# vLAR-group/unMORE

Hardware: NVIDIA B200
Metric: object_reasoning_images_per_sec (higher is better)
Workload: dtype f32

## Files before the change

include/unmore_b200.h:

```cpp
#ifndef UNMORE_B200_H_
#define UNMORE_B200_H_

#include <stddef.h>
#include <stdint.h>

#ifdef __cplusplus
extern "C" {
#endif

#define UNMORE_E_INVALID (-1)
#define UNMORE_E_CAPACITY (-2)

typedef void* unmore_stream_t;

const char* unmore_last_error(void);
int unmore_version(void);
size_t unmore_workspace_bytes(int n_img);

int unmore_existence_scores(const float* fields, int n_img, int C, int H, int W, int ch_exist,
                            const void* boxes, int boxes_f64, const int* counts, int cap,
                            float* scores_out, void* ws, unmore_stream_t stream);

int unmore_crop_resize(const float* fields, int n_img, int C, int H, int W,
                       const int* channels_host, int n_channels, const void* boxes, int boxes_f64,
// ... 16 lines not shown
                                     float max_sdf_thres, float max_shrink_threshold, float delta_ratio,
                                     float* boxes_out, float* labels_out, float* deltas_ws, float* max_ws,
                                     unmore_stream_t stream);
int unmore_score_and_rasterise_from_tiles(const float* tiles, const float* existence_scores, int antialias,
                                          int n_img, int H, int W, const void* boxes, int boxes_f64,
                                          const int* counts, int cap, float* scores_out, float* tight_out,
                                          int* areas_out, uint32_t* masks_out, unmore_stream_t stream);

int unmore_center_reasoning(const float* fields, int n_img, int C, int H, int W, int ch_sdf,
                            int ch_center_row, int ch_center_col, const void* boxes, int boxes_f64,
                            const int* counts, int cap, double center_score_max_thres,
                            double* max_values_out, int* argmax_out, double* splits_out,
                            unsigned char* cc_counts_out, double* cc_boxes_out, int* cc_overflow,
                            void* ws, unmore_stream_t stream);
int unmore_cc_cap(void);

int unmore_boundary_refine(const float* fields, int n_img, int C, int H, int W, int ch_sdf,
                           const void* boxes, int boxes_f64, const int* counts, int cap, int n_round,
                           int apply_small_filter, int early_exit, float proposal_area_thres,
                           float max_sdf_thres, float max_shrink_threshold, float delta_ratio,
                           float* boxes_out, float* labels_out, int* rounds_out, void* ws,
                           unmore_stream_t stream);

int unmore_existence_scores_aa(const float* fields, int n_img, int C, int H, int W, int ch_exist,
                               const void* boxes, int boxes_f64, const int* counts, int cap,
                               float* scores_out, void* ws, unmore_stream_t stream);
int unmore_boundary_refine_aa(const float* fields, int n_img, int C, int H, int W, int ch_sdf,
                              const void* boxes, int boxes_f64, const int* counts, int cap, int n_round,
                              int apply_small_filter, int early_exit, float proposal_area_thres,
                              float max_sdf_thres, float max_shrink_threshold, float delta_ratio,
// ... 74 lines not shown
```

unmore_b200/_lib.py:

```python
from __future__ import annotations

import ctypes as C
import os

_HERE = os.path.dirname(os.path.abspath(__file__))
LIB_PATH = os.environ.get("UNMORE_B200_LIB", os.path.join(_HERE, "libunmore_b200.so"))

_p = C.c_void_p
_i = C.c_int
_f = C.c_float
_d = C.c_double

SIGNATURES = {
    "unmore_existence_scores": [_p, _i, _i, _i, _i, _i, _p, _i, _p, _i, _p, _p, _p],
    "unmore_existence_scores_aa": [_p, _i, _i, _i, _i, _i, _p, _i, _p, _i, _p, _p, _p],
    "unmore_crop_resize": [_p, _i, _i, _i, _i, _p, _i, _p, _i, _p, _i, _p, _p],
    "unmore_crop_resize_aa": [_p, _i, _i, _i, _i, _p, _i, _p, _i, _p, _i, _p, _p, C.c_size_t, _p],
    "unmore_mask_resize_aa": [_p, _i, _i, _i, _i, _i, _p, _p, C.c_size_t, _p],
    "unmore_tile_means": [_p, C.c_longlong, _i, _p, _p],
    "unmore_center_reasoning_from_tiles": [_p, _i, _i, _i, _p, _i, _p, _i, _d, _p, _p, _p, _p, _p, _p, _p, _p],
    "unmore_boundary_round_from_tiles": [_p, _i, _p, _i, _i, _i, _f, _f, _f, _p, _p, _p, _p, _p],
    "unmore_score_and_rasterise_from_tiles": [_p, _p, _i, _i, _i, _i, _p, _i, _p, _i, _p, _p, _p, _p, _p],
    "unmore_center_reasoning": [_p, _i, _i, _i, _i, _i, _i, _i, _p, _i, _p, _i, _d, _p, _p, _p, _p, _p, _p, _p, _p],
    "unmore_boundary_refine": [_p, _i, _i, _i, _i, _i, _p, _i, _p, _i, _i, _i, _i, _f, _f, _f, _f, _p, _p, _p, _p, _p],
    "unmore_boundary_refine_aa": [_p, _i, _i, _i, _i, _i, _p, _i, _p, _i, _i, _i, _i, _f, _f, _f, _f, _p, _p, _p, _p, _p],
    "unmore_update_bbox_from_tiles": [_p, _i, _p, _p, _p],
    "unmore_compact_boxes": [_p, _i, _p, _i, _i, _i, _p, _f, _p, _i, _i, _p, _i, _p, _p, _p, _i, _p],
    "unmore_box_nms": [_p, _p, _p, _i, _i, _f, _p, _p, _p, _p, _p],
    "unmore_batch_erode": [_p, _i, _i, _i, _i, _i, _p, _p],
    "unmore_connected_components": [_p, _i, _i, _i, _p, _p, _p],
    "unmore_anti_center_map": [_p, _i, _i, _i, _i, _p, _p],
    "unmore_box_nms_matrix": [_p, _p, _i, _f, _p, _p, _p, _p, _p],
    "unmore_score_and_rasterise": [_p, _i, _i, _i, _i, _i, _i, _i, _i, _p, _i, _p, _i, _p, _p, _p, _p, _p],
    "unmore_mask_resize": [_p, _i, _i, _i, _i, _i, _p, _p],
    "unmore_final_scores": [_p, _p, _p, _p, _p, _i, _i, _d, _d, _d, _p, _p, _p, _p],
    "unmore_pack_detections": [_p, _p, _p, _p, _i, _i, _p, _i, _p],
    "unmore_sat_build": [_p, _i, _i, _i, _p, _p],
    "unmore_sat_build_fields": [_p, _i, _i, _i, _i, _p, _i, _p, _p],
# ... 43 lines not shown
```

unmore_b200/csrc/capi.cu:

```cuda
#include <cstdio>
#include <cstdarg>
#include <cmath>
#include <cstring>

#include "../../include/unmore_b200.h"
#include "unmore_internal.h"

using namespace unmore;

namespace {

thread_local char g_err[512] = "";

int fail(int code, const char* fmt, ...) {
  va_list ap;
  va_start(ap, fmt);
  vsnprintf(g_err, sizeof(g_err), fmt, ap);
  va_end(ap);
  return code;
}

int cuda_fail(int code, const char* what) {
  if (code == 0) return 0;
  snprintf(g_err, sizeof(g_err), "%s: %s", what, cudaGetErrorString((cudaError_t)code));
// ... 96 lines not shown
  if (int e = make_worklist(p.work, counts, n_img, cap, ws, s)) return e;
  if (W <= kWindowMaxSide && H <= kWindowMaxSide) {
    p.windows = window_tables(ws, n_img);
    const int e = (int)cudaMemsetAsync(p.windows, 0, sizeof(WindowSlot) * kWindowSlots * (size_t)n_img, s);
    if (e) return cuda_fail(e, "memset window tables");
  }
  if (aa) return cuda_fail(launch_refine_aa(p, num_sms(), s), "refine_aa_kernel");
  return cuda_fail(launch_refine(p, num_sms(), s), "refine_kernel");
}

}

extern "C" {

const char* unmore_last_error(void) { return g_err; }
int unmore_version(void) { return 101; }
size_t unmore_workspace_bytes(int n_img) {
  return worklist_bytes(n_img) + (n_img > 0 ? alignof(WindowSlot) - 1 + sizeof(WindowSlot) * kWindowSlots * (size_t)n_img : 0);
}

int unmore_existence_scores(const float* fields, int n_img, int C, int H, int W, int ch_exist, const void* boxes,
                            int boxes_f64, const int* counts, int cap, float* scores_out, void* ws,
                            unmore_stream_t stream) {
  return existence_scores("unmore_existence_scores", false, fields, n_img, C, H, W, ch_exist, boxes, boxes_f64, counts, cap,
                          scores_out, ws, (cudaStream_t)stream);
}

int unmore_existence_scores_aa(const float* fields, int n_img, int C, int H, int W, int ch_exist, const void* boxes,
                               int boxes_f64, const int* counts, int cap, float* scores_out, void* ws,
                               unmore_stream_t stream) {
  return existence_scores("unmore_existence_scores_aa", true, fields, n_img, C, H, W, ch_exist, boxes, boxes_f64, counts, cap,
// ... 49 lines not shown
      ch_center_row >= C || ch_center_col < 0 || ch_center_col >= C)
    return fail(UNMORE_E_INVALID, "unmore_center_reasoning: bad argument");
  if (cap == 0) return 0;
  cudaStream_t s = (cudaStream_t)stream;
  CenterParams p{};
  p.fields = fields; p.C = C; p.H = H; p.W = W;
  p.ch_sdf = ch_sdf; p.ch_crow = ch_center_row; p.ch_ccol = ch_center_col;
  p.boxes = boxes; p.boxes_f64 = boxes_f64; p.thr = center_score_max_thres;
  p.max_values = max_values_out; p.argmax = argmax_out; p.splits = splits_out;
  if ((cc_counts_out != nullptr) != (cc_boxes_out != nullptr) || (cc_counts_out != nullptr) != (cc_overflow != nullptr))
    return fail(UNMORE_E_INVALID, "unmore_center_reasoning: the three analyze_cc outputs go together");
  p.cc_counts = cc_counts_out; p.cc_boxes = cc_boxes_out; p.cc_overflow = cc_overflow;
  center_filters(p);
  if (int e = make_worklist(p.work, counts, n_img, cap, ws, s)) return e;
  return cuda_fail(launch_center(p, num_sms(), s), "center_kernel");
}

int unmore_boundary_refine(const float* fields, int n_img, int C, int H, int W, int ch_sdf, const void* boxes,
                           int boxes_f64, const int* counts, int cap, int n_round, int apply_small_filter,
                           int early_exit, float proposal_area_thres, float max_sdf_thres, float max_shrink_threshold,
                           float delta_ratio, float* boxes_out, float* labels_out, int* rounds_out, void* ws,
                           unmore_stream_t stream) {
  return boundary_refine("unmore_boundary_refine", false, fields, n_img, C, H, W, ch_sdf, boxes, boxes_f64, counts, cap, n_round,
                         apply_small_filter, early_exit, proposal_area_thres, max_sdf_thres, max_shrink_threshold,
                         delta_ratio, boxes_out, labels_out, rounds_out, ws, (cudaStream_t)stream);
}

int unmore_boundary_refine_aa(const float* fields, int n_img, int C, int H, int W, int ch_sdf, const void* boxes,
                              int boxes_f64, const int* counts, int cap, int n_round, int apply_small_filter,
                              int early_exit, float proposal_area_thres, float max_sdf_thres, float max_shrink_threshold,
// ... 249 lines not shown
```

unmore_b200/csrc/center.cu:

```cuda
#include "resample.cuh"
#include "unmore_internal.h"

namespace unmore {

constexpr int kCenterThreads = 256;
constexpr int kCenterWarps = kCenterThreads / 32;
constexpr int kWinLo = 10, kWinHi = 118, kWin = kWinHi - kWinLo;
constexpr int kWinStride = 110;
constexpr int kErode = 12;
constexpr int kCandCap = 1024;

struct CenterSmem {
  float2 c[kWin * kWinStride];
  uint32_t mask[kCrop][4];
  uint32_t hrun[kCrop][4];
  uint32_t ero[kCrop][4];
  double red_val[kCenterWarps];
  int red_idx[kCenterWarps];
  float red_f[kCenterWarps];
  float red_m[kCenterWarps];
  int bcast_i[2];
  int cc_scan[kCenterWarps];
  int cand_n;
  uint16_t cand[kCandCap];
// ... 158 lines not shown
};

struct CenterTileRows {
  const float* tile;
  __device__ __forceinline__ void row(int lane, int i, float s[4], f32x2 ab[4]) const {
    const float* r = tile + i * kCrop + lane;
#pragma unroll
    for (int c = 0; c < 4; ++c) {
      s[c] = __ldg(r + 32 * c);
      ab[c] = pk2(__ldg(r + kCrop * kCrop + 32 * c), __ldg(r + 2 * kCrop * kCrop + 32 * c));
    }
  }
};

constexpr int kSpecPlaneElems = 480 * 640;
template <bool ANALYZE_CC, int PLANE_ELEMS, bool ROW_SKIP>
__global__ void __launch_bounds__(kCenterThreads, 2) center_kernel(const CenterParams p) {
  extern __shared__ __align__(16) unsigned char smem_raw[];
  CenterSmem& sm = *reinterpret_cast<CenterSmem*>(smem_raw);
  struct WorkItem { int id, img, k, pad; double box[4]; };
  __shared__ __align__(16) WorkItem s_item[2];
  const int tid = threadIdx.x, lane = tid & 31, warp = tid >> 5;
  const int total = worklist_total(p.work);
  auto fetch_box = [&](int slot, int fimg, int fk) {
    const size_t frow = (size_t)fimg * p.work.cap + fk;
    const unsigned dst = smem_addr(&s_item[slot].box[0]);
    if (p.boxes_f64) {
      const char* src = reinterpret_cast<const char*>(p.boxes) + frow * 32;
      asm volatile("cp.async.ca.shared.global [%0], [%1], 16;" ::"r"(dst), "l"(src) : "memory");
      asm volatile("cp.async.ca.shared.global [%0], [%1], 16;" ::"r"(dst + 16), "l"(src + 16) : "memory");
    } else {
// ... 53 lines not shown
      const float scale_y = __fdiv_rn((float)win.h(), (float)kCrop);
      const int in_h = win.h();
      float cabs = 0.f;
      const bool col_in[4] = {lane >= kWinLo, true, true, lane + 96 < kWinHi};
      constexpr bool kLattice = ROW_SKIP && !ANALYZE_CC && PLANE_ELEMS >= 0;
      constexpr int kLatFirst = 8, kLatStride = 16, kLatRows = kCrop / kLatStride;
      constexpr int kRowsPerWarp = (kCrop + kCenterWarps - 1) / kCenterWarps;
      int i_begin, i_end, i_step;
      if constexpr (kLattice) { i_begin = kLatFirst + kLatStride * warp; i_end = kCrop; i_step = kLatStride * kCenterWarps; }
      else { i_begin = warp * kRowsPerWarp; i_end = min(kCrop, i_begin + kRowsPerWarp); i_step = 1; }
      int rmin = kErode, rmax = kCrop - kErode - 1;
      bool no_survivors = false;
      const unsigned stage_base = smem_addr(&sm.c[0]) + (unsigned)(((0 - kWinLo) * kWinStride + (lane - kWinLo)) * 8);
      const unsigned mask_base = smem_addr(&sm.mask[0][0]);
      const bool lane0 = lane == 0;
#pragma unroll 1
      for (int phase = 0; phase < (kLattice ? 2 : 1); ++phase) {
        const AxisTap my_tap = axis_tap(scale_y, min(i_begin + lane * i_step, kCrop - 1), in_h);
        int j = 0;
        for (int i = i_begin; i < i_end; i += i_step, ++j) {
          if (kLattice && phase == 1 && (i & (kLatStride - 1)) == kLatFirst) continue;
          const bool row_in = i >= kWinLo && i < kWinHi;
          const unsigned stage_addr = stage_base + (unsigned)(i * (kWinStride * 8));
          const unsigned mask_addr = mask_base + 16u * (unsigned)i;
          AxisTap v;
          v.i0 = __shfl_sync(kFullMask, my_tap.i0, j);
          v.l1 = __shfl_sync(kFullMask, my_tap.l1, j);
          v.i1 = min(v.i0 + 1, in_h - 1);
          v.l0 = __fsub_rn(1.f, v.l1);
          float s[4];
          f32x2 ab[4];
          if constexpr (PLANE_ELEMS < 0) trows.row(lane, i, s, ab);
          else rows.row(taps, v, s, ab);
          uint32_t word[4];
#pragma unroll
          for (int c = 0; c < 4; ++c) {
            float a2, b2;
            upk2(mul2(ab[c], ab[c]), a2, b2);
            const float sq = __fadd_rn(a2, b2);
            const bool on = (s[c] > UNMORE_SIGMOID_HALF_THRESHOLD) || (sq > UNMORE_NORM_HALF_SQ_THRESHOLD);
            word[c] = __ballot_sync(kFullMask, on);
            cabs = fmaxf(cabs, sq);
          }
          st_shared_b32_if<0>(lane0, mask_addr, word[0]);
          st_shared_b32_if<4>(lane0, mask_addr, word[1]);
          st_shared_b32_if<8>(lane0, mask_addr, word[2]);
          st_shared_b32_if<12>(lane0, mask_addr, word[3]);
          st_shared_b64_if<0>(row_in && col_in[0], stage_addr, ab[0]);
          st_shared_b64_if<256>(row_in, stage_addr, ab[1]);
          st_shared_b64_if<512>(row_in, stage_addr, ab[2]);
          st_shared_b64_if<768>(row_in && col_in[3], stage_addr, ab[3]);
        }
        if (kLattice && phase == 0) {
          __syncthreads();
          bool alive_row = false;
          if (lane < kLatRows) {
            u128 m = load_row(sm.mask[kLatFirst + kLatStride * lane]);
            m &= m >> 1; m &= m >> 2; m &= m >> 4; m &= m >> 8; m &= m >> 9;
            alive_row = m != 0;
          }
          const unsigned alive = __ballot_sync(kFullMask, alive_row);
          unsigned long long klo = 0, khi = 0;
#pragma unroll
          for (int k = 0; k < kLatRows; ++k) {
            const int l = kLatFirst + kLatStride * k, a = l - kErode < 0 ? 0 : l - kErode, b = l + kErode > kCrop - 1 ? kCrop - 1 : l + kErode;
            unsigned long long lo = 0, hi = 0;
// ... 20 lines not shown
        m &= m >> 1; m &= m >> 2; m &= m >> 4; m &= m >> 8;
        m &= m >> 9;
        store_row(sm.hrun[tid], m << kErode);
      }
      __syncthreads();
      if (tid < kCrop) {
        u128 e = 0;
        if (tid >= rmin && tid <= rmax) {
          e = ~(u128)0;
#pragma unroll 5
          for (int d = -kErode; d <= kErode; ++d) e &= load_row(sm.hrun[tid + d]);
        }
        store_row(sm.ero[tid], e);
      }
      __syncthreads();
      constexpr int kInner = kCrop - 2 * kErode;
      constexpr int kStrips = kInner / 8;
      constexpr int kMaxOwn = (kInner * kStrips + kCenterThreads - 1) / kCenterThreads;
      float own_max[kMaxOwn];
      auto strip_bits = [&](int r, int k) -> uint32_t {
        const int c = kErode + 8 * k;
        const uint32_t lo = sm.ero[r][c >> 5], hi = sm.ero[r][min((c >> 5) + 1, 3)];
        return (__funnelshift_r(lo, hi, c & 31)) & 0xffu;
      };
      auto strip_scores = [&](int r, int k, float acc[8]) {
        f32x2 acc2[8];
#pragma unroll
        for (int x = 0; x < 8; ++x) acc2[x] = pk2(0.f, 0.f);
        const int c = kErode + 8 * k;
#pragma unroll
        for (int di = 0; di < 5; ++di) {
          const int o = (r + di - 2 - kWinLo) * kWinStride + (c - 2 - kWinLo);
          f32x2 v[12];
#pragma unroll
          for (int q2 = 0; q2 < 6; ++q2) {
            const ulonglong2 t = *reinterpret_cast<const ulonglong2*>(&sm.c[o + 2 * q2]);
            v[2 * q2] = t.x; v[2 * q2 + 1] = t.y;
          }
#pragma unroll
          for (int dj = 0; dj < 5; ++dj) {
            if (di == 2 && dj == 2) continue;
            const f32x2 f = p.filt_pair[di * 5 + dj];
#pragma unroll
            for (int x = 0; x < 8; ++x) acc2[x] = fma2(f, v[x + dj], acc2[x]);
          }
        }
#pragma unroll
        for (int x = 0; x < 8; ++x) {
          float lo, hi;
          upk2(acc2[x], lo, hi);
          acc[x] = lo + hi;
        }
      };
      float m32 = -INFINITY;
#pragma unroll
      for (int m = 0; m < kMaxOwn; ++m) {
        own_max[m] = -INFINITY;
        const int q = tid + m * kCenterThreads;
        if (q < kInner * kStrips) {
          const int r = kErode + q % kInner, k = q / kInner;
          const uint32_t bits = strip_bits(r, k);
          if (bits) {
            float acc[8];
            strip_scores(r, k, acc);
#pragma unroll
            for (int x = 0; x < 8; ++x)
              if ((bits >> x) & 1u) own_max[m] = fmaxf(own_max[m], acc[x]);
            m32 = fmaxf(m32, own_max[m]);
// ... 19 lines not shown
        if (!any_cand || !(own_max[m] >= cand_thr)) continue;
        const int q = tid + m * kCenterThreads;
        const int r = kErode + q % kInner, k = q / kInner;
        const uint32_t bits = strip_bits(r, k);
        float acc[8];
        strip_scores(r, k, acc);
#pragma unroll
        for (int x = 0; x < 8; ++x) {
          if (((bits >> x) & 1u) && acc[x] >= cand_thr) {
            const int slot = atomicAdd(&sm.cand_n, 1);
            if (slot < kCandCap) sm.cand[slot] = (uint16_t)(r * kCrop + kErode + 8 * k + x);
          }
        }
      }
      __syncthreads();
      auto exact = [&](int r, int c) -> double {
        double e = 0.0;
#pragma unroll
        for (int di = 0; di < 5; ++di) {
#pragma unroll
          for (int dj = 0; dj < 5; ++dj) {
            if (di == 2 && dj == 2) continue;
            const float2 cc = sm.c[(r + di - 2 - kWinLo) * kWinStride + (c + dj - 2 - kWinLo)];
            e = fma(p.filt[di * 5 + dj], (double)cc.x, e);
            e = fma(p.filt[dj * 5 + di], (double)cc.y, e);
          }
        }
        return __ddiv_rn(e, 24.0);
      };
      double tbest = 0.0;
      int tidx = -1;
      const int n_cand = sm.cand_n;
      if (n_cand <= kCandCap) {
        for (int q = tid; q < n_cand; q += kCenterThreads) {
          const int flat = sm.cand[q];
          const double e = exact(flat >> 7, flat & (kCrop - 1));
          if (tidx < 0 || e > tbest || (e == tbest && flat < tidx)) { tbest = e; tidx = flat; }
        }
      } else {
#pragma unroll 1
        for (int m = 0; m < kMaxOwn; ++m) {
          if (!(own_max[m] >= cand_thr)) continue;
          const int q = tid + m * kCenterThreads;
          const int r = kErode + q % kInner, k = q / kInner;
// ... 18 lines not shown
      }
      if (lane == 0) { sm.red_val[warp] = tbest; sm.red_idx[warp] = tidx; }
      __syncthreads();
      if (warp == 0) {
        double ov = lane < kCenterWarps ? sm.red_val[lane] : 0.0;
        int oi = lane < kCenterWarps ? sm.red_idx[lane] : -1;
#pragma unroll
        for (int o = 16; o > 0; o >>= 1) {
          const double pv = __shfl_xor_sync(kFullMask, ov, o);
          const int pi = __shfl_xor_sync(kFullMask, oi, o);
          if (pi >= 0 && (oi < 0 || pv > ov || (pv == ov && pi < oi))) { ov = pv; oi = pi; }
        }
        best = ov; best_idx = oi;
      }
      }
    }
    if (tid == 0) {
      const double maxv = (best_idx >= 0 && best > 0.0) ? best : 0.0;
      const bool pass = maxv <= p.thr;
      sm.bcast_i[0] = pass ? 1 : 0;
      p.max_values[row] = maxv;
      p.argmax[row] = pass ? -1 : best_idx;
      if (!pass && p.splits) {
        const int yc = best_idx / kCrop, xc = best_idx % kCrop;
        const double xr = (double)((float)xc / (float)kCrop), yr = (double)((float)yc / (float)kCrop);
        const double xs = __dadd_rn(x1, __dmul_rn(__dsub_rn(x2, x1), xr));
        const double ys = __dadd_rn(y1, __dmul_rn(__dsub_rn(y2, y1), yr));
        double* o = p.splits + row * 16;
        o[0] = x1; o[1] = y1; o[2] = xs; o[3] = y2;
        o[4] = xs; o[5] = y1; o[6] = x2; o[7] = y2;
        o[8] = x1; o[9] = y1; o[10] = x2; o[11] = ys;
        o[12] = x1; o[13] = ys; o[14] = x2; o[15] = y2;
      }
    }
    if constexpr (ANALYZE_CC) {
      __syncthreads();
      int n_comp = 0;
      if (sm.bcast_i[0] && !win.empty()) {
// ... 127 lines not shown
  if (tid == 0) counts[b] = n;
  if (tid < min(n, kCcCap)) {
    int* o = boxes + ((size_t)b * kCcCap + tid) * 4;
    o[0] = sm.box[0][tid]; o[1] = sm.box[1][tid]; o[2] = sm.box[2][tid] + 1; o[3] = sm.box[3][tid] + 1;
  }
}

int launch_components(const unsigned char* masks, int B, int* counts, int* boxes, cudaStream_t stream) {
  if (B <= 0) return 0;
  cudaError_t e = cudaFuncSetAttribute(components_kernel, cudaFuncAttributeMaxDynamicSharedMemorySize, (int)sizeof(CcSmem));
  if (e != cudaSuccess) return (int)e;
  components_kernel<<<B, kCenterThreads, sizeof(CcSmem), stream>>>(masks, B, counts, boxes);
  return (int)cudaGetLastError();
}

template <bool CC, int PE, bool RS = false>
static int launch_center_t(const CenterParams& p, int num_sms, cudaStream_t stream) {
  cudaError_t e = cudaFuncSetAttribute(center_kernel<CC, PE, RS>, cudaFuncAttributeMaxDynamicSharedMemorySize, (int)sizeof(CenterSmem));
  if (e != cudaSuccess) return (int)e;
  center_kernel<CC, PE, RS><<<num_sms * 2, kCenterThreads, sizeof(CenterSmem), stream>>>(p);
  return (int)cudaGetLastError();
}

int launch_center(const CenterParams& p, int num_sms, cudaStream_t stream) {
  if (p.tiles) return p.cc_counts ? launch_center_t<true, -1>(p, num_sms, stream) : launch_center_t<false, -1>(p, num_sms, stream);
  const bool spec = p.H * p.W == kSpecPlaneElems && p.ch_crow == p.ch_sdf + 1 && p.ch_ccol == p.ch_sdf + 2;
  if (p.cc_counts) return spec ? launch_center_t<true, kSpecPlaneElems>(p, num_sms, stream) : launch_center_t<true, 0>(p, num_sms, stream);
  if (p.splits)
    return spec ? launch_center_t<false, kSpecPlaneElems, true>(p, num_sms, stream) : launch_center_t<false, 0, true>(p, num_sms, stream);
  return spec ? launch_center_t<false, kSpecPlaneElems>(p, num_sms, stream) : launch_center_t<false, 0>(p, num_sms, stream);
}

}
```

unmore_b200/csrc/unmore_internal.h:

```cpp
#pragma once
#include <cuda_runtime.h>
#include <stdint.h>

#include "common.cuh"

namespace unmore {

constexpr int kWindowSlots = 32768;
static_assert((kWindowSlots & (kWindowSlots - 1)) == 0, "kWindowSlots must be a power of two");
constexpr int kWindowMaxSide = 32767;
struct alignas(32) WindowSlot {
  unsigned long long key;
  float max_sdf, pad;
  float4 d;
};
static_assert(sizeof(WindowSlot) == 32, "one sector per slot");

struct RefineParams {
  const float* fields;
  int C, H, W, ch_sdf;
  const void* boxes;
  int boxes_f64;
  WorkList work;
  int n_round;
// ... 40 lines not shown
  const float* tiles;
  const float* fields;
  int C, H, W, ch_sdf, ch_crow, ch_ccol;
  const void* boxes;
  int boxes_f64;
  WorkList work;
  double thr;
  double* max_values;
  int* argmax;
  double* splits;
  double filt[25];
  unsigned long long filt_pair[25];
  unsigned char* cc_counts;
  double* cc_boxes;
  int* cc_overflow;
};
int launch_center(const CenterParams& p, int num_sms, cudaStream_t stream);
int launch_components(const unsigned char* masks, int B, int* counts, int* boxes, cudaStream_t stream);
int launch_erode(const unsigned char* in, unsigned char* out, int B, int kernel_size, int num_round, cudaStream_t stream);
int launch_anti_center(const float* vote, double* out, int B, int H, int W, const double* filt25, cudaStream_t stream);

int launch_prefix_counts(const int* counts, int n_img, int* offsets, cudaStream_t stream);

enum CompactMode { kFlagsU8 = 0, kScoreGE = 1, kLabelEQ = 2, kArgmaxGE0 = 3, kArgmaxLT0 = 4 };
struct CompactParams {
  const void* in;
  int in_f64;
  const int* counts_in;
  int cap_in;
  int group;
// ... 77 lines not shown
```

unmore_b200/object_reasoning.py:

```python
from __future__ import annotations

import argparse
import json
import os
from typing import Dict, Optional

import numpy as np
import torch

from . import ops
from .synth import anchor_proposals

HYPER_DEFAULTS = dict(
    class_score_thres=0.1, center_score_max_thres=0.009, analyze_cc=False, max_sdf_thres=0.5,
    max_shrink_threshold=16, delta_ratio=0.5, n_round=50, proposal_area_thres=50, seed=0)


def default_args(**over) -> argparse.Namespace:
    d = dict(HYPER_DEFAULTS)
    d.update(over)
    return argparse.Namespace(**d)


def _label_boxes_host(mask_u8: np.ndarray):
# ... 358 lines not shown
                for b in range(B):
                    n = c1h[b]
                    if n == 0 or int((cc_counts[b, :n] >= capc).sum()) == 0:
                        continue
                    passing = torch.nonzero(am1[b, :n] < 0).flatten().tolist()
                    extra = self._cc_boxes_with_overflow(fields[b:b + 1], p1[b:b + 1], passing, cc_counts[b], cc_boxes[b],
                                                         fields.shape[-2], fields.shape[-1])
                    n_split = 4 * int((am1[b, :n] >= 0).sum())
                    if n_split + len(extra) > split_cap:
                        raise RuntimeError("analyze_cc: component boxes exceeded the split-list capacity")
                    split[b, n_split:n_split + len(extra)] = torch.as_tensor(extra, device=dev)
                    sc[b] = n_split + len(extra)
        ex2 = ops.existence_scores(fields, split, sc, ch=ch, ws=ws, antialias=aa)
        p2, c2, _ = ops.compact_boxes(split, sc, ops.MODE_SCORE_GE, ex2, thr=a.class_score_thres, out_dtype=f64)
        _, am2, _, _ = ops.center_reasoning(fields, p2, c2, thr=a.center_score_max_thres, ch=ch, ws=ws, want_splits=False,
                                            antialias=aa)
        ops.compact_boxes(p2, c2, ops.MODE_ARGMAX_LT0, am2, out=refine_in, counts_out=rc, append=True)
        rb, lab, rounds = ops.boundary_refine(fields, refine_in, rc, n_round=a.n_round, apply_small_filter=True,
                                              early_exit=True, proposal_area_thres=a.proposal_area_thres,
                                              max_sdf_thres=a.max_sdf_thres,
                                              max_shrink_threshold=a.max_shrink_threshold, delta_ratio=a.delta_ratio,
                                              ch=ch, ws=ws, want_rounds=stats is not None, antialias=aa)
        lost1 = torch.zeros((1,), dtype=torch.int32, device=dev) if cap_out > 32768 else None
        fin, fc, _ = ops.compact_boxes(rb, rc, ops.MODE_LABEL_EQ, lab, thr=1.0, out_dtype=torch.float32,
                                       cap_out=min(cap_out, 32768), overflow=lost1)
        if lost1 is not None and int(lost1.item()):
            raise RuntimeError("more than 32768 label-1 boxes in one image")
        _, kc, kb = ops.box_nms(fin, None, fc, iou_threshold=0.5)
        if stats is not None:
            stats.update(existence_in=counts, pass1=c1, split=sc, split_kept=c2, refine_in=rc, refine_rounds=rounds,
                         label1=fc, kept=kc, existence_scores=ex, refine_boxes=rb, refine_labels=lab,
# ... 27 lines not shown
```

unmore_b200/ops.py:

```python
from __future__ import annotations

import threading
from dataclasses import dataclass
from typing import Optional, Tuple

import torch

from . import _lib
from .synth import CH_CCOL, CH_CROW, CH_EXIST, CH_SDF

CROP = 128


@dataclass(frozen=True)
class Channels:
    sdf: int = CH_SDF
    center_row: int = CH_CROW
    center_col: int = CH_CCOL
    exist: int = CH_EXIST


DEFAULT_CHANNELS = Channels()


# ... 30 lines not shown
        self.launches += kernels

    def summary(self):
        torch.cuda.synchronize()
        out = {}
        for name, a, b in self.events:
            d = out.setdefault(name, {"ms": 0.0, "calls": 0})
            d["ms"] += a.elapsed_time(b)
            d["calls"] += 1
        return out


_timer: Optional[StageTimer] = None
LAUNCHES = 0

_KERNELS = {"unmore_crop_resize": 1, "unmore_crop_resize_aa": 2, "unmore_mask_resize_aa": 2, "unmore_existence_scores": 1, "unmore_center_reasoning": 1, "unmore_boundary_refine": 1,
            "unmore_existence_scores_aa": 1, "unmore_boundary_refine_aa": 1,
            "unmore_update_bbox_from_tiles": 1, "unmore_compact_boxes": 1, "unmore_box_nms": 1,
            "unmore_batch_erode": 1, "unmore_anti_center_map": 1, "unmore_connected_components": 1, "unmore_box_nms_matrix": 3,
            "unmore_score_and_rasterise": 1, "unmore_mask_resize": 1, "unmore_final_scores": 1, "unmore_sat_build": 1, "unmore_sat_build_fields": 1, "unmore_box_sums": 1,
            "unmore_mask_pack": 1, "unmore_mask_stats": 1, "unmore_mask_nms": 3, "unmore_mask_rle_counts": 1,
            "unmore_pack_detections": 1, "unmore_tile_means": 1, "unmore_center_reasoning_from_tiles": 1,
            "unmore_boundary_round_from_tiles": 2, "unmore_score_and_rasterise_from_tiles": 1}


def set_timer(t: Optional[StageTimer]):
    global _timer
    _timer = t


def _call(name, *args, counts=None):
    global LAUNCHES
    k = _KERNELS[name] + (1 if counts is not None else 0)
    LAUNCHES += k
    dev = _cur_device()
    try:
        if dev is not None and dev.index is not None and dev.index != torch.cuda.current_device():
            with torch.cuda.device(dev):
                _lib.call(name, *args) if _timer is None else _timer.record(name, k, _lib.call, *args)
        elif _timer is not None:
            _timer.record(name, k, _lib.call, *args)
        else:
            _lib.call(name, *args)
    finally:
        _tls.device = None


def _ptr(t: Optional[torch.Tensor]):
    return None if t is None else t.data_ptr()


def _check_fields(fields: torch.Tensor) -> Tuple[int, int, int, int]:
    if not fields.is_cuda:
        raise _lib.UnmoreError("fields must live on a CUDA device (no CPU path)")
    if fields.dtype != torch.float32 or fields.dim() != 4 or not fields.is_contiguous():
        raise _lib.UnmoreError("fields must be contiguous fp32 [n_img, C, H, W]")
# ... 50 lines not shown
            _on(fields)
            _call("unmore_crop_resize_aa", fields.data_ptr(), n_img, C, H, W, ctypes.cast(ch, ctypes.c_void_p), len(channels),
                  bsl.data_ptr(), f64, _ptr(cnt), c1 - c0, osl.data_ptr(), scratch.data_ptr(), scratch.numel() * 4, _stream())
            out[:, c0:c1] = osl
        return out
    if cap:
        _call("unmore_crop_resize", fields.data_ptr(), n_img, C, H, W, ctypes.cast(ch, ctypes.c_void_p), len(channels),
              boxes.data_ptr(), f64, _ptr(counts), cap, out.data_ptr(), _stream())
    return out


CENTER_AA_SLICE_BYTES = 1 << 30


def center_reasoning(fields, boxes, counts=None, thr: float = 0.009, ch: Channels = DEFAULT_CHANNELS, ws=None,
                     want_splits: bool = True, analyze_cc: bool = False, antialias: bool = False):
    n_img, C, H, W = _check_fields(fields)
    cap, f64 = _check_boxes(boxes, n_img)
    _check_counts(counts, n_img)
    dev = fields.device
    ws = workspace(n_img, dev) if ws is None else ws
    if antialias:
        return _center_reasoning_aa(fields, boxes, counts, thr, ch, ws, want_splits, analyze_cc)
    maxv = torch.zeros((n_img, cap), dtype=torch.float64, device=dev)
    argmax = torch.full((n_img, cap), -1, dtype=torch.int32, device=dev)
    splits = torch.zeros((n_img, cap, 4, 4), dtype=torch.float64, device=dev) if want_splits else None
    cc = None
    if analyze_cc:
        cc_cap = _lib.load().unmore_cc_cap()
        cc = (torch.zeros((n_img, cap), dtype=torch.uint8, device=dev),
              torch.zeros((n_img, cap, cc_cap, 4), dtype=torch.float64, device=dev),
              torch.zeros((1,), dtype=torch.int32, device=dev))
    _call("unmore_center_reasoning", fields.data_ptr(), n_img, C, H, W, ch.sdf, ch.center_row, ch.center_col,
          boxes.data_ptr(), f64, _ptr(counts), cap, float(thr), maxv.data_ptr(), argmax.data_ptr(),
          _ptr(splits), _ptr(cc[0]) if cc else None, _ptr(cc[1]) if cc else None, _ptr(cc[2]) if cc else None,
          ws.data_ptr(), _stream(), counts=counts)
# ... 378 lines not shown
```

Baseline: 2084.

## Add banded early-exit decision kernel for second-pass center reasoning

Adds a decision-only variant of the center kernel that stages the crop in 64-row bands and, after each band, erodes, screens candidates and checks the exact score against the threshold. It stops as soon as any pixel passes. The second center-reasoning call in the pipeline, whose splits are unused, now takes this path when antialiasing is off, so rows past the first passing band are never resized or scored. The cost is extra per-band synchronisation and a new template instantiation. Its result (max value, argmax) may differ from the full pass, since it stops at the first band with a passing pixel rather than scanning the whole crop.

```diff
diff --git a/include/unmore_b200.h b/include/unmore_b200.h
--- a/include/unmore_b200.h
+++ b/include/unmore_b200.h
@@ -54,6 +54,11 @@
                             unsigned char* cc_counts_out, double* cc_boxes_out, int* cc_overflow,
                             void* ws, unmore_stream_t stream);
 int unmore_cc_cap(void);
+
+int unmore_center_decide(const float* fields, int n_img, int C, int H, int W, int ch_sdf, int ch_center_row,
+                         int ch_center_col, const void* boxes, int boxes_f64, const int* counts, int cap,
+                         double center_score_max_thres, double* max_values_out, int* argmax_out, void* ws,
+                         unmore_stream_t stream);
 
 int unmore_boundary_refine(const float* fields, int n_img, int C, int H, int W, int ch_sdf,
                            const void* boxes, int boxes_f64, const int* counts, int cap, int n_round,
diff --git a/unmore_b200/_lib.py b/unmore_b200/_lib.py
--- a/unmore_b200/_lib.py
+++ b/unmore_b200/_lib.py
@@ -22,6 +22,7 @@
     "unmore_boundary_round_from_tiles": [_p, _i, _p, _i, _i, _i, _f, _f, _f, _p, _p, _p, _p, _p],
     "unmore_score_and_rasterise_from_tiles": [_p, _p, _i, _i, _i, _i, _p, _i, _p, _i, _p, _p, _p, _p, _p],
     "unmore_center_reasoning": [_p, _i, _i, _i, _i, _i, _i, _i, _p, _i, _p, _i, _d, _p, _p, _p, _p, _p, _p, _p, _p],
+    "unmore_center_decide": [_p, _i, _i, _i, _i, _i, _i, _i, _p, _i, _p, _i, _d, _p, _p, _p, _p],
     "unmore_boundary_refine": [_p, _i, _i, _i, _i, _i, _p, _i, _p, _i, _i, _i, _i, _f, _f, _f, _f, _p, _p, _p, _p, _p],
     "unmore_boundary_refine_aa": [_p, _i, _i, _i, _i, _i, _p, _i, _p, _i, _i, _i, _i, _f, _f, _f, _f, _p, _p, _p, _p, _p],
     "unmore_update_bbox_from_tiles": [_p, _i, _p, _p, _p],
diff --git a/unmore_b200/csrc/capi.cu b/unmore_b200/csrc/capi.cu
--- a/unmore_b200/csrc/capi.cu
+++ b/unmore_b200/csrc/capi.cu
@@ -134,7 +134,7 @@
 extern "C" {
 
 const char* unmore_last_error(void) { return g_err; }
-int unmore_version(void) { return 101; }
+int unmore_version(void) { return 102; }
 size_t unmore_workspace_bytes(int n_img) {
   return worklist_bytes(n_img) + (n_img > 0 ? alignof(WindowSlot) - 1 + sizeof(WindowSlot) * kWindowSlots * (size_t)n_img : 0);
 }
@@ -214,6 +214,26 @@
   center_filters(p);
   if (int e = make_worklist(p.work, counts, n_img, cap, ws, s)) return e;
   return cuda_fail(launch_center(p, num_sms(), s), "center_kernel");
+}
+
+int unmore_center_decide(const float* fields, int n_img, int C, int H, int W, int ch_sdf, int ch_center_row,
+                         int ch_center_col, const void* boxes, int boxes_f64, const int* counts, int cap,
+                         double center_score_max_thres, double* max_values_out, int* argmax_out, void* ws,
+                         unmore_stream_t stream) {
+  if (int e = check_fields(fields, n_img, C, H, W)) return e;
+  if (!boxes || !max_values_out || !argmax_out || !ws || cap < 0 || ch_sdf < 0 || ch_sdf >= C || ch_center_row < 0 ||
+      ch_center_row >= C || ch_center_col < 0 || ch_center_col >= C)
+    return fail(UNMORE_E_INVALID, "unmore_center_decide: bad argument");
+  if (cap == 0) return 0;
+  cudaStream_t s = (cudaStream_t)stream;
+  CenterParams p{};
+  p.fields = fields; p.C = C; p.H = H; p.W = W;
+  p.ch_sdf = ch_sdf; p.ch_crow = ch_center_row; p.ch_ccol = ch_center_col;
+  p.boxes = boxes; p.boxes_f64 = boxes_f64; p.thr = center_score_max_thres;
+  p.max_values = max_values_out; p.argmax = argmax_out; p.decide = 1;
+  center_filters(p);
+  if (int e = make_worklist(p.work, counts, n_img, cap, ws, s)) return e;
+  return cuda_fail(launch_center(p, num_sms(), s), "center_kernel (decide)");
 }
 
 int unmore_boundary_refine(const float* fields, int n_img, int C, int H, int W, int ch_sdf, const void* boxes,
diff --git a/unmore_b200/csrc/center.cu b/unmore_b200/csrc/center.cu
--- a/unmore_b200/csrc/center.cu
+++ b/unmore_b200/csrc/center.cu
@@ -196,7 +196,8 @@
 };
 
 constexpr int kSpecPlaneElems = 480 * 640;
-template <bool ANALYZE_CC, int PLANE_ELEMS, bool ROW_SKIP>
+constexpr int kDecideBand = 64;
+template <bool ANALYZE_CC, int PLANE_ELEMS, bool ROW_SKIP, bool DECIDE = false>
 __global__ void __launch_bounds__(kCenterThreads, 2) center_kernel(const CenterParams p) {
   extern __shared__ __align__(16) unsigned char smem_raw[];
   CenterSmem& sm = *reinterpret_cast<CenterSmem*>(smem_raw);
@@ -280,25 +281,19 @@
       const unsigned stage_base = smem_addr(&sm.c[0]) + (unsigned)(((0 - kWinLo) * kWinStride + (lane - kWinLo)) * 8);
       const unsigned mask_base = smem_addr(&sm.mask[0][0]);
       const bool lane0 = lane == 0;
-#pragma unroll 1
-      for (int phase = 0; phase < (kLattice ? 2 : 1); ++phase) {
-        const AxisTap my_tap = axis_tap(scale_y, min(i_begin + lane * i_step, kCrop - 1), in_h);
-        int j = 0;
-        for (int i = i_begin; i < i_end; i += i_step, ++j) {
-          if (kLattice && phase == 1 && (i & (kLatStride - 1)) == kLatFirst) continue;
+      auto stage_row = [&](auto& src, const ColTaps& tp, int i, const AxisTap& tap, int j, uint32_t word[4]) {
           const bool row_in = i >= kWinLo && i < kWinHi;
           const unsigned stage_addr = stage_base + (unsigned)(i * (kWinStride * 8));
           const unsigned mask_addr = mask_base + 16u * (unsigned)i;
           AxisTap v;
-          v.i0 = __shfl_sync(kFullMask, my_tap.i0, j);
-          v.l1 = __shfl_sync(kFullMask, my_tap.l1, j);
+          v.i0 = __shfl_sync(kFullMask, tap.i0, j);
+          v.l1 = __shfl_sync(kFullMask, tap.l1, j);
           v.i1 = min(v.i0 + 1, in_h - 1);
           v.l0 = __fsub_rn(1.f, v.l1);
           float s[4];
           f32x2 ab[4];
           if constexpr (PLANE_ELEMS < 0) trows.row(lane, i, s, ab);
-          else rows.row(taps, v, s, ab);
-          uint32_t word[4];
+          else src.row(tp, v, s, ab);
 #pragma unroll
           for (int c = 0; c < 4; ++c) {
             float a2, b2;
@@ -316,6 +311,188 @@
           st_shared_b64_if<256>(row_in, stage_addr, ab[1]);
           st_shared_b64_if<512>(row_in, stage_addr, ab[2]);
           st_shared_b64_if<768>(row_in && col_in[3], stage_addr, ab[3]);
+      };
+      constexpr int kInner = kCrop - 2 * kErode;
+      constexpr int kStrips = kInner / 8;
+      auto strip_bits = [&](int r, int k) -> uint32_t {
+        const int c = kErode + 8 * k;
+        const uint32_t lo = sm.ero[r][c >> 5], hi = sm.ero[r][min((c >> 5) + 1, 3)];
+        return (__funnelshift_r(lo, hi, c & 31)) & 0xffu;
+      };
+      auto strip_scores = [&](int r, int k, float acc[8]) {
+        f32x2 acc2[8];
+#pragma unroll
+        for (int x = 0; x < 8; ++x) acc2[x] = pk2(0.f, 0.f);
+        const int c = kErode + 8 * k;
+#pragma unroll
+        for (int di = 0; di < 5; ++di) {
+          const int o = (r + di - 2 - kWinLo) * kWinStride + (c - 2 - kWinLo);
+          f32x2 v[12];
+#pragma unroll
+          for (int q2 = 0; q2 < 6; ++q2) {
+            const ulonglong2 t = *reinterpret_cast<const ulonglong2*>(&sm.c[o + 2 * q2]);
+            v[2 * q2] = t.x; v[2 * q2 + 1] = t.y;
+          }
+#pragma unroll
+          for (int dj = 0; dj < 5; ++dj) {
+            if (di == 2 && dj == 2) continue;
+            const f32x2 f = p.filt_pair[di * 5 + dj];
+#pragma unroll
+            for (int x = 0; x < 8; ++x) acc2[x] = fma2(f, v[x + dj], acc2[x]);
+          }
+        }
+#pragma unroll
+        for (int x = 0; x < 8; ++x) {
+          float lo, hi;
+          upk2(acc2[x], lo, hi);
+          acc[x] = lo + hi;
+        }
+      };
+      auto exact = [&](int r, int c) -> double {
+        double e = 0.0;
+#pragma unroll
+        for (int di = 0; di < 5; ++di) {
+#pragma unroll
+          for (int dj = 0; dj < 5; ++dj) {
+            if (di == 2 && dj == 2) continue;
+            const float2 cc = sm.c[(r + di - 2 - kWinLo) * kWinStride + (c + dj - 2 - kWinLo)];
+            e = fma(p.filt[di * 5 + dj], (double)cc.x, e);
+            e = fma(p.filt[dj * 5 + di], (double)cc.y, e);
+          }
+        }
+        return __ddiv_rn(e, 24.0);
+      };
+      if constexpr (DECIDE) {
+      static_assert(PLANE_ELEMS >= 0, "the decision form reads the fields");
+      constexpr int kDecideRows = kDecideBand / kCenterWarps;
+      constexpr int kBands = kCrop / kDecideBand;
+      constexpr int kBandOwn = (kDecideBand * kStrips + kCenterThreads - 1) / kCenterThreads;
+      static_assert(kDecideRows * kBands <= 32, "one vertical tap per lane");
+      const AxisTap my_tap = axis_tap(
+          scale_y, ((lane / kDecideRows) % kBands) * kDecideBand + warp * kDecideRows + lane % kDecideRows, in_h);
+      const float thr_acc = __double2float_rd(__dmul_rn(p.thr, 24.0));
+      int lo = kErode;
+#pragma unroll 1
+      for (int b = 0; b < kBands; ++b) {
+        ColTaps btaps;
+        btaps.init<kStrided>(lane, win.w());
+        CenterRows<(PLANE_ELEMS > 0 ? PLANE_ELEMS : 0)> brows;
+        brows.init(planes, p.W, win);
+        for (int rr = 0; rr < kDecideRows; ++rr) {
+          const int i = b * kDecideBand + warp * kDecideRows + rr;
+          uint32_t word[4];
+          stage_row(brows, btaps, i, my_tap, b * kDecideRows + rr, word);
+          u128 m = ((u128)word[3] << 96) | ((u128)word[2] << 64) | ((u128)word[1] << 32) | (u128)word[0];
+          m &= m >> 1; m &= m >> 2; m &= m >> 4; m &= m >> 8;
+          m &= m >> 9;
+          if (lane0) store_row(sm.hrun[i], m << kErode);
+        }
+        const int hi = (b + 1) * kDecideBand - 1 - kErode;
+        if (hi < lo) continue;
+        const float wmax = warp_max(cabs);
+        if (lane0) sm.red_f[warp] = wmax;
+        __syncthreads();
+        locate_next();
+        const int n = hi - lo + 1;
+        if (tid < n) {
+          const int r = lo + tid;
+          u128 e = ~(u128)0;
+#pragma unroll 5
+          for (int d = -kErode; d <= kErode; ++d) e &= load_row(sm.hrun[r + d]);
+          store_row(sm.ero[r], e);
+        }
+        if (tid == kCenterThreads - 1) sm.cand_n = 0;
+        float cmax = 0.f;
+#pragma unroll
+        for (int w = 0; w < kCenterWarps; ++w) cmax = fmaxf(cmax, sm.red_f[w]);
+        __syncthreads();
+        cmax = __fmul_rn(__fsqrt_ru(cmax), 1.000001f);
+        const float margin = 8.0f * 48.0f * 5.9604645e-08f * 31.0f * cmax;
+        const float cand_thr = __fsub_rd(thr_acc, margin);
+        bool queued = false;
+#pragma unroll
+        for (int mo = 0; mo < kBandOwn; ++mo) {
+          const int q = tid + mo * kCenterThreads;
+          if (q < n * kStrips) {
+            const int r = lo + q % n, k = q / n;
+            const uint32_t bits = strip_bits(r, k);
+            if (bits) {
+              float acc[8];
+              strip_scores(r, k, acc);
+#pragma unroll
+              for (int x = 0; x < 8; ++x) {
+                if (((bits >> x) & 1u) && acc[x] >= cand_thr) {
+                  const int slot = atomicAdd(&sm.cand_n, 1);
+                  if (slot < kCandCap) sm.cand[slot] = (uint16_t)(r * kCrop + kErode + 8 * k + x);
+                  queued = true;
+                }
+              }
+            }
+          }
+        }
+        if (__syncthreads_or(queued)) {
+          double tbest = 0.0;
+          int tidx = -1;
+          const int n_cand = sm.cand_n;
+          if (n_cand <= kCandCap) {
+            for (int q = tid; q < n_cand; q += kCenterThreads) {
+              const int flat = sm.cand[q];
+              const double e = exact(flat >> 7, flat & (kCrop - 1));
+              if (e > p.thr && (tidx < 0 || e > tbest || (e == tbest && flat < tidx))) { tbest = e; tidx = flat; }
+            }
+          } else {
+#pragma unroll 1
+            for (int mo = 0; mo < kBandOwn; ++mo) {
+              const int q = tid + mo * kCenterThreads;
+              if (q >= n * kStrips) break;
+              const int r = lo + q % n, k = q / n;
+              const uint32_t bits = strip_bits(r, k);
+              if (!bits) continue;
+              float acc[8];
+              strip_scores(r, k, acc);
+#pragma unroll 1
+              for (int x = 0; x < 8; ++x) {
+                if (!((bits >> x) & 1u) || !(acc[x] >= cand_thr)) continue;
+                const int c = kErode + 8 * k + x;
+                const double e = exact(r, c);
+                const int flat = r * kCrop + c;
+                if (e > p.thr && (tidx < 0 || e > tbest || (e == tbest && flat < tidx))) { tbest = e; tidx = flat; }
+              }
+            }
+          }
+#pragma unroll
+          for (int o = 16; o > 0; o >>= 1) {
+            const double ov = __shfl_xor_sync(kFullMask, tbest, o);
+            const int oi = __shfl_xor_sync(kFullMask, tidx, o);
+            if (oi >= 0 && (tidx < 0 || ov > tbest || (ov == tbest && oi < tidx))) { tbest = ov; tidx = oi; }
+          }
+          if (lane0) { sm.red_val[warp] = tbest; sm.red_idx[warp] = tidx; }
+          if (__syncthreads_or(tidx >= 0)) {
+            if (warp == 0) {
+              double ov = lane < kCenterWarps ? sm.red_val[lane] : 0.0;
+              int oi = lane < kCenterWarps ? sm.red_idx[lane] : -1;
+#pragma unroll
+              for (int o = 16; o > 0; o >>= 1) {
+                const double pv = __shfl_xor_sync(kFullMask, ov, o);
+                const int pi = __shfl_xor_sync(kFullMask, oi, o);
+                if (pi >= 0 && (oi < 0 || pv > ov || (pv == ov && pi < oi))) { ov = pv; oi = pi; }
+              }
+              best = ov; best_idx = oi;
+            }
+            break;
+          }
+        }
+        lo = hi + 1;
+      }
+      } else {
+#pragma unroll 1
+      for (int phase = 0; phase < (kLattice ? 2 : 1); ++phase) {
+        const AxisTap my_tap = axis_tap(scale_y, min(i_begin + lane * i_step, kCrop - 1), in_h);
+        int j = 0;
+        for (int i = i_begin; i < i_end; i += i_step, ++j) {
+          if (kLattice && phase == 1 && (i & (kLatStride - 1)) == kLatFirst) continue;
+          uint32_t word[4];
+          stage_row(rows, taps, i, my_tap, j, word);
         }
         if (kLattice && phase == 0) {
           __syncthreads();
@@ -366,44 +543,8 @@
         store_row(sm.ero[tid], e);
       }
       __syncthreads();
-      constexpr int kInner = kCrop - 2 * kErode;
-      constexpr int kStrips = kInner / 8;
       constexpr int kMaxOwn = (kInner * kStrips + kCenterThreads - 1) / kCenterThreads;
       float own_max[kMaxOwn];
-      auto strip_bits = [&](int r, int k) -> uint32_t {
-        const int c = kErode + 8 * k;
-        const uint32_t lo = sm.ero[r][c >> 5], hi = sm.ero[r][min((c >> 5) + 1, 3)];
-        return (__funnelshift_r(lo, hi, c & 31)) & 0xffu;
-      };
-      auto strip_scores = [&](int r, int k, float acc[8]) {
-        f32x2 acc2[8];
-#pragma unroll
-        for (int x = 0; x < 8; ++x) acc2[x] = pk2(0.f, 0.f);
-        const int c = kErode + 8 * k;
-#pragma unroll
-        for (int di = 0; di < 5; ++di) {
-          const int o = (r + di - 2 - kWinLo) * kWinStride + (c - 2 - kWinLo);
-          f32x2 v[12];
-#pragma unroll
-          for (int q2 = 0; q2 < 6; ++q2) {
-            const ulonglong2 t = *reinterpret_cast<const ulonglong2*>(&sm.c[o + 2 * q2]);
-            v[2 * q2] = t.x; v[2 * q2 + 1] = t.y;
-          }
-#pragma unroll
-          for (int dj = 0; dj < 5; ++dj) {
-            if (di == 2 && dj == 2) continue;
-            const f32x2 f = p.filt_pair[di * 5 + dj];
-#pragma unroll
-            for (int x = 0; x < 8; ++x) acc2[x] = fma2(f, v[x + dj], acc2[x]);
-          }
-        }
-#pragma unroll
-        for (int x = 0; x < 8; ++x) {
-          float lo, hi;
-          upk2(acc2[x], lo, hi);
-          acc[x] = lo + hi;
-        }
-      };
       float m32 = -INFINITY;
 #pragma unroll
       for (int m = 0; m < kMaxOwn; ++m) {
@@ -453,20 +594,6 @@
         }
       }
       __syncthreads();
-      auto exact = [&](int r, int c) -> double {
-        double e = 0.0;
-#pragma unroll
-        for (int di = 0; di < 5; ++di) {
-#pragma unroll
-          for (int dj = 0; dj < 5; ++dj) {
-            if (di == 2 && dj == 2) continue;
-            const float2 cc = sm.c[(r + di - 2 - kWinLo) * kWinStride + (c + dj - 2 - kWinLo)];
-            e = fma(p.filt[di * 5 + dj], (double)cc.x, e);
-            e = fma(p.filt[dj * 5 + di], (double)cc.y, e);
-          }
-        }
-        return __ddiv_rn(e, 24.0);
-      };
       double tbest = 0.0;
       int tidx = -1;
       const int n_cand = sm.cand_n;
@@ -515,6 +642,7 @@
         best = ov; best_idx = oi;
       }
       }
+      }
     }
     if (tid == 0) {
       const double maxv = (best_idx >= 0 && best > 0.0) ? best : 0.0;
@@ -522,7 +650,7 @@
       sm.bcast_i[0] = pass ? 1 : 0;
       p.max_values[row] = maxv;
       p.argmax[row] = pass ? -1 : best_idx;
-      if (!pass && p.splits) {
+      if (!DECIDE && !pass && p.splits) {
         const int yc = best_idx / kCrop, xc = best_idx % kCrop;
         const double xr = (double)((float)xc / (float)kCrop), yr = (double)((float)yc / (float)kCrop);
         const double xs = __dadd_rn(x1, __dmul_rn(__dsub_rn(x2, x1), xr));
@@ -680,11 +808,11 @@
   return (int)cudaGetLastError();
 }
 
-template <bool CC, int PE, bool RS = false>
+template <bool CC, int PE, bool RS = false, bool DECIDE = false>
 static int launch_center_t(const CenterParams& p, int num_sms, cudaStream_t stream) {
-  cudaError_t e = cudaFuncSetAttribute(center_kernel<CC, PE, RS>, cudaFuncAttributeMaxDynamicSharedMemorySize, (int)sizeof(CenterSmem));
+  cudaError_t e = cudaFuncSetAttribute(center_kernel<CC, PE, RS, DECIDE>, cudaFuncAttributeMaxDynamicSharedMemorySize, (int)sizeof(CenterSmem));
   if (e != cudaSuccess) return (int)e;
-  center_kernel<CC, PE, RS><<<num_sms * 2, kCenterThreads, sizeof(CenterSmem), stream>>>(p);
+  center_kernel<CC, PE, RS, DECIDE><<<num_sms * 2, kCenterThreads, sizeof(CenterSmem), stream>>>(p);
   return (int)cudaGetLastError();
 }
 
@@ -694,6 +822,9 @@
   if (p.cc_counts) return spec ? launch_center_t<true, kSpecPlaneElems>(p, num_sms, stream) : launch_center_t<true, 0>(p, num_sms, stream);
   if (p.splits)
     return spec ? launch_center_t<false, kSpecPlaneElems, true>(p, num_sms, stream) : launch_center_t<false, 0, true>(p, num_sms, stream);
+  if (p.decide && p.thr >= 0.0)
+    return spec ? launch_center_t<false, kSpecPlaneElems, false, true>(p, num_sms, stream)
+                : launch_center_t<false, 0, false, true>(p, num_sms, stream);
   return spec ? launch_center_t<false, kSpecPlaneElems>(p, num_sms, stream) : launch_center_t<false, 0>(p, num_sms, stream);
 }
 
diff --git a/unmore_b200/csrc/unmore_internal.h b/unmore_b200/csrc/unmore_internal.h
--- a/unmore_b200/csrc/unmore_internal.h
+++ b/unmore_b200/csrc/unmore_internal.h
@@ -78,6 +78,7 @@
   unsigned char* cc_counts;
   double* cc_boxes;
   int* cc_overflow;
+  int decide;
 };
 int launch_center(const CenterParams& p, int num_sms, cudaStream_t stream);
 int launch_components(const unsigned char* masks, int B, int* counts, int* boxes, cudaStream_t stream);
diff --git a/unmore_b200/object_reasoning.py b/unmore_b200/object_reasoning.py
--- a/unmore_b200/object_reasoning.py
+++ b/unmore_b200/object_reasoning.py
@@ -396,7 +396,7 @@
         ex2 = ops.existence_scores(fields, split, sc, ch=ch, ws=ws, antialias=aa)
         p2, c2, _ = ops.compact_boxes(split, sc, ops.MODE_SCORE_GE, ex2, thr=a.class_score_thres, out_dtype=f64)
         _, am2, _, _ = ops.center_reasoning(fields, p2, c2, thr=a.center_score_max_thres, ch=ch, ws=ws, want_splits=False,
-                                            antialias=aa)
+                                            antialias=aa, decision_only=not aa)
         ops.compact_boxes(p2, c2, ops.MODE_ARGMAX_LT0, am2, out=refine_in, counts_out=rc, append=True)
         rb, lab, rounds = ops.boundary_refine(fields, refine_in, rc, n_round=a.n_round, apply_small_filter=True,
                                               early_exit=True, proposal_area_thres=a.proposal_area_thres,
diff --git a/unmore_b200/ops.py b/unmore_b200/ops.py
--- a/unmore_b200/ops.py
+++ b/unmore_b200/ops.py
@@ -68,7 +68,7 @@
 _timer: Optional[StageTimer] = None
 LAUNCHES = 0
 
-_KERNELS = {"unmore_crop_resize": 1, "unmore_crop_resize_aa": 2, "unmore_mask_resize_aa": 2, "unmore_existence_scores": 1, "unmore_center_reasoning": 1, "unmore_boundary_refine": 1,
+_KERNELS = {"unmore_crop_resize": 1, "unmore_crop_resize_aa": 2, "unmore_mask_resize_aa": 2, "unmore_existence_scores": 1, "unmore_center_reasoning": 1, "unmore_center_decide": 1, "unmore_boundary_refine": 1,
             "unmore_existence_scores_aa": 1, "unmore_boundary_refine_aa": 1,
             "unmore_update_bbox_from_tiles": 1, "unmore_compact_boxes": 1, "unmore_box_nms": 1,
             "unmore_batch_erode": 1, "unmore_anti_center_map": 1, "unmore_connected_components": 1, "unmore_box_nms_matrix": 3,
@@ -83,7 +83,7 @@
     _timer = t
 
 
-def _call(name, *args, counts=None):
+def _call(name, *args, counts=None, stage=None):
     global LAUNCHES
     k = _KERNELS[name] + (1 if counts is not None else 0)
     LAUNCHES += k
@@ -91,9 +91,9 @@
     try:
         if dev is not None and dev.index is not None and dev.index != torch.cuda.current_device():
             with torch.cuda.device(dev):
-                _lib.call(name, *args) if _timer is None else _timer.record(name, k, _lib.call, *args)
+                _lib.call(name, *args) if _timer is None else _timer.record(stage or name, k, lambda _, *a: _lib.call(name, *a), *args)
         elif _timer is not None:
-            _timer.record(name, k, _lib.call, *args)
+            _timer.record(stage or name, k, lambda _, *a: _lib.call(name, *a), *args)
         else:
             _lib.call(name, *args)
     finally:
@@ -174,12 +174,22 @@
 
 
 def center_reasoning(fields, boxes, counts=None, thr: float = 0.009, ch: Channels = DEFAULT_CHANNELS, ws=None,
-                     want_splits: bool = True, analyze_cc: bool = False, antialias: bool = False):
+                     want_splits: bool = True, analyze_cc: bool = False, antialias: bool = False,
+                     decision_only: bool = False):
     n_img, C, H, W = _check_fields(fields)
     cap, f64 = _check_boxes(boxes, n_img)
     _check_counts(counts, n_img)
     dev = fields.device
     ws = workspace(n_img, dev) if ws is None else ws
+    if decision_only:
+        if want_splits or analyze_cc or antialias:
+            raise ValueError("center_reasoning: decision_only takes want_splits=False, analyze_cc=False, antialias=False")
+        maxv = torch.zeros((n_img, cap), dtype=torch.float64, device=dev)
+        argmax = torch.full((n_img, cap), -1, dtype=torch.int32, device=dev)
+        _call("unmore_center_decide", fields.data_ptr(), n_img, C, H, W, ch.sdf, ch.center_row, ch.center_col,
+              boxes.data_ptr(), f64, _ptr(counts), cap, float(thr), maxv.data_ptr(), argmax.data_ptr(), ws.data_ptr(),
+              _stream(), counts=counts, stage="unmore_center_reasoning")
+        return maxv, argmax, None, None
     if antialias:
         return _center_reasoning_aa(fields, boxes, counts, thr, ch, ws, want_splits, analyze_cc)
     maxv = torch.zeros((n_img, cap), dtype=torch.float64, device=dev)
```

New measurement: 2068, median of 6. About the same (-0.8%).
